# chechaohp/gan-ode

Measured on AMD Instinct MI355X. Metric: generated videos/sec (16-frame clips), higher is better.
Workload: dtype f32

## Files before the change

### gan-ode_amd/_lib.py

```python
from __future__ import annotations

import ctypes as C
import os
import sys

_HERE = os.path.dirname(os.path.abspath(__file__))
LIB_PATH = os.path.join(_HERE, "lib", "libgode.so")

i32, i64, f32, ptr = C.c_int32, C.c_int64, C.c_float, C.c_void_p
cint, u32, u64 = C.c_int, C.c_uint32, C.c_uint64

ACT_NONE, ACT_RELU, ACT_LRELU, ACT_TANH_OUT = 0, 1, 2, 3
ACT_TANH, ACT_SIGMOID = 4, 5
ACT_LRELU01 = 6
EPI_RAW, EPI_TANH = 0, 1
FPROP, DGRAD = 0, 1
PACK_BORDER = 0x100
OP_IGEMM, OP_WGRAD, OP_BN_FINALIZE, OP_BN_BWD, OP_ODE_FWD, OP_ODE_BWD, OP_BCE, OP_ADAM, OP_PACK = range(1, 10)
OP_ODERNN_FWD, OP_ODERNN_BWD, OP_BN_APPLY, OP_COL2IM = 10, 11, 12, 13
OP_SDE_FWD, OP_SDE_BWD = 14, 15
OP_CDE_FWD, OP_CDE_BWD = 16, 17
OP_WGAN = 18
OP_GRU_FWD, OP_GRU_BWD = 19, 20
OP_DNOISE = 21
# ... 37 lines not shown

class ConvGeom(C.Structure):
    _fields_ = [(n, i32) for n in "N Ci Co Di Hi Wi Do Ho Wo kd kh kw sd sh sw pd ph pw".split()]

    def key(self):
        return tuple(getattr(self, n) for n, _ in self._fields_)


class _Op(C.Structure):
    """An op of gode_run (a GODE_OPS row of gode.h): a subclass names its kind and its `int FN(const op*, stream)` entry
    point once; _STRUCTS, the prototypes, EXPORTS and run_one's dispatch all follow from the subclasses."""


class IgemmOp(_Op):
    _fields_ = [("g", ConvGeom), ("dir", i32), ("act", i32), ("epilogue", i32), ("tile", i32), ("src", ptr),
                ("wpack", ptr), ("out", ptr), ("scale", ptr), ("shift", ptr), ("stats", ptr), ("gs", i64 * 5),
                ("work", ptr), ("groups", i32), ("border", i32)]
    KIND, FN = OP_IGEMM, "gode_igemm"


class WgradOp(_Op):
    _fields_ = [("g", ConvGeom), ("act", i32), ("xform_on_y", i32), ("splits", i32), ("accumulate", i32),
                ("x", ptr), ("y", ptr), ("scale", ptr), ("shift", ptr), ("work", ptr), ("dw", ptr),
                ("co_perm", ptr), ("co_canon", i64), ("xs", i64 * 5)]
    KIND, FN = OP_WGRAD, "gode_wgrad"


class BnFinalizeOp(_Op):
    _fields_ = [("stats", ptr), ("rows", i32), ("ncols", i32), ("C", i32), ("count", i64), ("gamma", ptr),
                ("beta", ptr), ("running_mean", ptr), ("running_var", ptr), ("num_batches_tracked", ptr),
                ("mean", ptr), ("invstd", ptr), ("scale", ptr), ("shift", ptr), ("momentum", f32), ("eps", f32),
                ("training", i32), ("pad_", i32), ("groups", i32), ("rows0", i32), ("nseg", i32), ("order", i32),
                ("count1", i64), ("seg", i32 * 24), ("stats1", ptr), ("rows1", i32), ("pad3_", i32), ("batch_var", ptr)]
    KIND, FN = OP_BN_FINALIZE, "gode_bn_finalize"


class BnRunningLayer(C.Structure):
    _fields_ = [("mean", ptr), ("var", ptr), ("running_mean", ptr), ("running_var", ptr), ("num_batches_tracked", ptr),
                ("C", i32), ("pad_", i32)]


class BnRunningOp(_Op):
    _fields_ = [("layer", BnRunningLayer * BN_RUNNING_MAX), ("n", i32), ("momentum", f32)]
    KIND, FN = OP_BN_RUNNING, "gode_bn_running"


class BnBwdOp(_Op):
# ... 267 lines not shown


_OPS = _Op.__subclasses__()
_STRUCTS = {0: ConvGeom, REC_ADAM_NOISE: AdamNoiseTensor, OP_PACK: PackOp, **{st.KIND: st for st in _OPS}}

_PROTOS = {
    "gode_igemm_stats_rows": ([ptr], cint),
    "gode_igemm_stats_rows0": ([ptr], cint),
    "gode_igemm_stats_segments": ([ptr, i32, ptr], cint),
    "gode_igemm_model_cycles": ([ptr], C.c_double),
    "gode_igemm_family": ([ptr], cint),
    "gode_igemm_dead_taps": ([ptr], C.c_double),
    "gode_igemm_launch_info": ([ptr, ptr], cint),
    "gode_igemm_launch_cell": ([ptr, ptr], cint),
    "gode_igemm_work_size": ([ptr], i64),
    "gode_col2im_launch_kind": ([ptr, ptr], cint),
    "gode_video_grid_launch_kind": ([ptr, ptr], cint),
    "gode_gif_lzw_bound": ([i64], i64),
    "gode_gif_lzw": ([ptr, i64, i32, ptr, i64], i64),
    "gode_pack_size": ([ptr, cint], i64),
    "gode_pack_weights": ([ptr, cint, ptr, ptr, ptr, i32, ptr], cint),
    "gode_wgrad_work_size": ([ptr], i64),
    "gode_wgrad_auto_splits": ([ptr], cint),
    "gode_bn_bwd_work_size": ([i64, i32], i64),
    "gode_ode_bwd_work_size": ([i32], i64),
    "gode_odernn_bwd_work_size": ([i32], i64),
    "gode_odernn_sync_size": ([i32], i64),
    "gode_sde_bwd_work_size": ([i32], i64),
    "gode_cde_sync_size": ([i32], i64),
    "gode_cde_state_size": ([i32, i32], i64),
    "gode_cde_bwd_work_size": ([i32], i64),
    "gode_gru_bwd_work_size": ([i32], i64),
    "gode_ode_fwd_multi": ([ptr, i32, ptr], cint),
    "gode_ode_bwd_multi": ([ptr, i32, ptr], cint),
    "gode_odernn_fwd_multi": ([ptr, i32, ptr], cint),
    "gode_odernn_bwd_multi": ([ptr, i32, ptr], cint),
    "gode_odernn_fwd_route": ([ptr, i32, ptr], cint),
    "gode_odernn_bwd_route": ([ptr, i32, ptr], cint),
    "gode_gru_fwd_multi": ([ptr, i32, ptr], cint),
    "gode_gru_bwd_multi": ([ptr, i32, ptr], cint),
    "gode_chstats_rows": ([i64], cint),
    "gode_cbn_bwd_work_size": ([i32, i32, i32, i32], i64),
    "gode_gres_out_bwd_work_size": ([i32, i32, i32, i32, i32, i32], i64),
    "gode_fc_act_bwd_work_size": ([i64, i32], i64),
    "gode_dropout_mask": ([ptr, i64, u64, u32, f32, ptr], cint),
    "gode_scale": ([ptr, ptr, i64, f32, cint, ptr], cint),
# ... 167 lines not shown
```

### gan-ode_amd/csrc/wgrad.hip

```cpp
#include "common.h"
#include "wgrad_plan.h"

struct WgradArgs {
  gode_conv_geom g;
  const float* x; const float* y; const float* scale; const float* shift; float* work;
  int32_t xsN, xsD, xsH, xsW, xsC;
  int32_t act, xform_on_y;
  int32_t M, chunk, Kt, taps;
  FastDiv dWo, dHo, dDo;
  uint32_t x_bytes;
};

template <int WM, int WN, int TM, int TN, bool VECX, bool VECY>
__global__ void __launch_bounds__(WM* WN * 64) wgrad_kernel(const WgradArgs a) {
  constexpr int NT = WM * WN * 64, BI = WM * TM * 32, BJ = WN * TN * 32;
  static_assert(NT == 256, "loader assumes 256 threads");
  constexpr int YC = BI / 4, XC = BJ / 4;
  constexpr int YR = NT / YC, XR = NT / XC;
  constexpr int YP = 32 / YR, XP = 32 / XR;
  static_assert(YP >= 1 && XP >= 1, "tile too narrow for the loader");
  __shared__ __attribute__((aligned(16))) float smem[2 * 32 * (BI + BJ)];

  const int tid = threadIdx.x, lane = tid & 63, wave = tid >> 6;
  const int wm = wave / WN, wn = wave % WN;
// ... 329 lines not shown
      stage();
      __syncthreads();
      fetch(s + 1);
      mma_slab(0);
      __syncthreads();
    }
    stage();
    __syncthreads();
    mma_slab(0);
  }

  float* dst = a.work + (int64_t)z * g.Co * a.Kt;
  const int col0 = jblk * BJ + wn * TN * 32 + (lane & 31) * TN;
#pragma unroll
  for (int i = 0; i < TM; ++i)
#pragma unroll
    for (int r = 0; r < 16; ++r) {
      const int row = iblk * BI + wm * TM * 32 + TM * ((r & 3) + 8 * (r >> 2) + 4 * (lane >> 5)) + i;
      if (row < g.Co && col0 < a.Kt) {
        bv_t v;
#pragma unroll
        for (int j = 0; j < TN; ++j) v[j] = acc[i][j][r];
        *reinterpret_cast<bv_t*>(dst + (int64_t)row * a.Kt + col0) = v;
      }
    }
}

__global__ void __launch_bounds__(256) wgrad_thin_kernel(const WgradArgs a, int chunk_thin) {
  const gode_conv_geom& g = a.g;
  const int C4 = g.Co >> 2;
  const int CL = C4 < 64 ? C4 : 64;
  const int ML = 256 / CL;
  const int tid = threadIdx.x, cl = tid % CL, ml = tid / CL;
  const int Kt = a.Kt;
  __shared__ __attribute__((aligned(16))) float red[4][256][4];
  const float nslope = gode_act_neg_slope(a.act);
  const float xneg = a.xform_on_y ? 1.f : nslope, yneg = a.xform_on_y ? nslope : 1.f;
  const int m0 = blockIdx.x * chunk_thin;
  const int m1 = m0 + chunk_thin < a.M ? m0 + chunk_thin : a.M;
  for (int cg = 0; cg < C4; cg += CL) {
    const int c4 = cg + cl;
    const bool cok = ml < ML && c4 < C4;
    f32x4 acc[THIN_MAXKT];
#pragma unroll
    for (int j = 0; j < THIN_MAXKT; ++j) acc[j] = f32x4{0.f, 0.f, 0.f, 0.f};
    f32x4 ysc = {1, 1, 1, 1}, ysh = {0, 0, 0, 0};
// ... 261 lines not shown
#pragma unroll 8
    for (int zz = 0; zz < splits; ++zz) {
      if (VEC4) {
        const f32x4 v = *reinterpret_cast<const f32x4*>(work + (int64_t)zz * total + i);
#pragma unroll
        for (int e = 0; e < V; ++e) sd[e] += (double)v[e];
      } else {
        sd[0] += (double)work[(int64_t)zz * total + i];
      }
    }
    int co = (int)(i / Kt);
    const int j0 = (int)(i - (int64_t)co * Kt);
    if (co_perm) { co = co_perm[co]; if (co < 0) continue; }
#pragma unroll
    for (int e = 0; e < V; ++e) {
      const int j = j0 + e, tap = j / Ci, ci = j - tap * Ci;
      float* dptr = dw + ((int64_t)co * Ci + ci) * taps + tap;
      const float sv = (float)sd[e];
      *dptr = accumulate ? *dptr + sv : sv;
    }
  }
}

#define RS_LANES 16
__global__ void __launch_bounds__(256) wgrad_reduce_small_kernel(const float* work, float* dw, int Co, int Ci, int taps,
                                                                 int splits, const int32_t* co_perm, int accumulate) {
  __shared__ double red[RS_LANES][RS_OUT];
  const int Kt = Ci * taps, total = Co * Kt;
  const int o = threadIdx.x & (RS_OUT - 1), ln = threadIdx.x / RS_OUT;
  const int i = blockIdx.x * RS_OUT + o;
  double sd = 0.0;
  if (i < total) {
#pragma unroll 8
    for (int zz = ln; zz < splits; zz += RS_LANES) sd += (double)work[(int64_t)zz * total + i];
  }
  red[ln][o] = sd;
  __syncthreads();
  if (ln == 0 && i < total) {
    double tot = 0.0;
#pragma unroll
    for (int q = 0; q < RS_LANES; ++q) tot += red[q][o];
    const float sv = (float)tot;
    int co = i / Kt;
    const int j = i - co * Kt, tap = j / Ci, ci = j - tap * Ci;
    if (co_perm) { co = co_perm[co]; if (co < 0) return; }
    float* dptr = dw + ((int64_t)co * Ci + ci) * taps + tap;
    *dptr = accumulate ? *dptr + sv : sv;
  }
}


extern "C" int gode_wgrad_auto_splits(const gode_conv_geom* g) { return wgrad_auto_splits(*g); }
extern "C" int64_t gode_wgrad_work_size(const gode_wgrad_op* op) { return wgrad_work_size(op); }

#define WG_TILE_ARGS(t) WGRAD_TILES[t].WM, WGRAD_TILES[t].WN, WGRAD_TILES[t].TM, WGRAD_TILES[t].TN

extern "C" int gode_wgrad(const gode_wgrad_op* op, void* stream) {
  if (!op || !op->x || !op->y || !op->work || !op->dw) return GODE_E_ARG;
  WgradPlan P;
  const int rc = wgrad_make_plan(op, &P);
  if (rc) return rc;
  const gode_conv_geom& g = op->g;
  const WgradPatch& w = P.work.patch;
  const int splits = P.work.splits;
  WpArgs WP;
  WgradArgs& A = WP.w;
  A.g = g; A.x = op->x; A.y = op->y; A.scale = op->scale; A.shift = op->shift; A.work = op->work;
  A.xsN = P.xs[0]; A.xsD = P.xs[1]; A.xsH = P.xs[2]; A.xsW = P.xs[3]; A.xsC = P.xs[4];
  A.act = op->act; A.xform_on_y = op->xform_on_y;
  A.M = P.M; A.chunk = P.chunk; A.Kt = P.Kt; A.taps = P.taps;
  A.dWo = make_fastdiv(g.Wo); A.dHo = make_fastdiv(g.Ho); A.dDo = make_fastdiv(g.Do);
  A.x_bytes = P.x_bytes;
  if (P.path == WG_PATCH) {
    WP.RB = w.RB; WP.CB = w.CB; WP.PR = w.PR; WP.PL = w.PL; WP.LW = w.LW; WP.nseg = w.nseg; WP.dseg = make_fastdiv((uint32_t)w.nseg);
    WP.segs = w.segs; WP.segs_per_wg = w.segs_per_wg; WP.yvec = P.vy;
  }
  hipStream_t st = (hipStream_t)stream;
  const dim3 grid(P.grid_x, P.grid_y, P.grid_z), block(P.block);
#define WG_CASE_FAST(t, gl) case wgrad_fast_key(t, gl): hipLaunchKernelGGL((wgrad_fast_kernel<WG_TILE_ARGS(t), gl != 0>), grid, block, 0, st, A); break;
#define WG_CASE_GENERIC(t, vx, vy) case wgrad_generic_key(t, vx, vy): hipLaunchKernelGGL((wgrad_kernel<WG_TILE_ARGS(t), vx != 0, vy != 0>), grid, block, 0, st, A); break;
#define WG_CASE_PATCH(n, c) case wgrad_patch_key(n, c): hipLaunchKernelGGL((wgrad_patch_kernel<n, c>), grid, block, P.lds_bytes, st, WP); break;
  switch (wgrad_kernel_key(P, g.Co)) {
    WGRAD_FAST_KERNELS(WG_CASE_FAST)
    WGRAD_GENERIC_KERNELS(WG_CASE_GENERIC)
    WGRAD_PATCH_KERNELS(WG_CASE_PATCH)
    case wgrad_thin_key(): hipLaunchKernelGGL(wgrad_thin_kernel, grid, block, 0, st, A, P.chunk_thin); break;
    default: return GODE_E_SHAPE;
  }
#undef WG_CASE_FAST
#undef WG_CASE_GENERIC
#undef WG_CASE_PATCH
  GODE_LAUNCH_CHECK();
  const dim3 rgrid(P.reduce_blocks), rblock(256);
  switch (P.reduce) {
    case WG_REDUCE_SMALL:
      hipLaunchKernelGGL(wgrad_reduce_small_kernel, rgrid, rblock, 0, st, op->work, op->dw, g.Co, g.Ci, P.taps, splits, op->co_perm, op->accumulate);
      break;
    case WG_REDUCE_VEC4:
      hipLaunchKernelGGL((wgrad_reduce_kernel<true>), rgrid, rblock, 0, st, op->work, op->dw, g.Co, g.Ci, P.taps, splits, op->co_perm, op->accumulate);
      break;
    default:
      hipLaunchKernelGGL((wgrad_reduce_kernel<false>), rgrid, rblock, 0, st, op->work, op->dw, g.Co, g.Ci, P.taps, splits, op->co_perm, op->accumulate);
  }
  GODE_LAUNCH_CHECK();
  return 0;
}
```

### gan-ode_amd/csrc/wgrad_plan.h

```cpp
#pragma once
#include <stdint.h>
#include <stdlib.h>
#include "conv_geom.h"

#define THIN_MAXKT 16
#define WP_MAXB 4
#define WP_MAXE 16
#define RS_OUT 16

enum { WG_TILE_32x128 = 0, WG_TILE_64x128 = 1, WG_TILE_128x128 = 2, WG_TILE_256x128 = 3, WG_TILE_128x256 = 4, WGRAD_TILE_IDS = 5 };
struct WgradTile { int BI, BJ, WM, WN, TM, TN, waves; };
constexpr WgradTile wgrad_tile(int WM, int WN, int TM, int TN) { return WgradTile{WM * TM * 32, WN * TN * 32, WM, WN, TM, TN, WM * WN}; }
static constexpr WgradTile WGRAD_TILES[WGRAD_TILE_IDS] = {wgrad_tile(1, 4, 1, 1), wgrad_tile(2, 2, 1, 2), wgrad_tile(2, 2, 2, 2),
                                                          wgrad_tile(4, 2, 2, 2), wgrad_tile(2, 4, 2, 2)};

struct WgradKnobs { int tile; bool generic, glds; };
static const WgradKnobs& wgrad_knobs() {
  static const WgradKnobs k = [] {
    const char* t = getenv("GODE_WGRAD_TILE");
    const char* gl = getenv("GODE_WGRAD_GLDS");
    return WgradKnobs{t ? atoi(t) : 0, getenv("GODE_WGRAD_GENERIC") != nullptr, gl ? atoi(gl) != 0 : true};
  }();
  return k;
}
// ... 55 lines not shown
  const int nseg = (g.Wo + 31) / 32;
  const int64_t segs = (int64_t)g.N * g.Do * g.Ho * nseg;
  if (segs >= (1ll << 31)) return false;
  int wgs = (int)(segs / 2 < 1 ? 1 : segs / 2);
  if (wgs > 512) wgs = 512;
  *P = WgradPatch{RB, CB, PR, PL, LW, nseg, (int)segs, (int)((segs + wgs - 1) / wgs), nbw};
  return true;
}

enum { WG_PATCH = 0, WG_THIN = 1, WG_GEMM = 2 };
struct WgradWork { int32_t rule, split_tile, splits; WgradPatch patch; };
static WgradWork wgrad_plan_work(const gode_conv_geom& g, int splits, bool has_scale, bool xform_on_y, const WgradKnobs& knobs) {
  WgradWork W = {WG_GEMM, wgrad_pick_tile(g, knobs), splits, {0, 0, 0, 0, 0, 0, 0, 0, 0}};
  if (wgrad_patch_shape(g, splits > 0, has_scale && !xform_on_y, &W.patch)) {
    W.rule = WG_PATCH; W.splits = (W.patch.segs + W.patch.segs_per_wg - 1) / W.patch.segs_per_wg;
  } else if (splits <= 0 && wgrad_thin_eligible(g)) {
    W.rule = WG_THIN; W.splits = wgrad_thin_blocks(g);
  } else if (splits <= 0) {
    W.splits = wgrad_gemm_splits(g, W.split_tile);
  }
  return W;
}
static int wgrad_auto_splits(const gode_conv_geom& g) { return wgrad_gemm_splits(g, wgrad_pick_tile(g, wgrad_knobs())); }
static int64_t wgrad_work_size(const gode_wgrad_op* op) {
  const WgradWork W = wgrad_plan_work(op->g, op->splits, op->scale != nullptr, op->xform_on_y != 0, wgrad_knobs());
  return (int64_t)W.splits * op->g.Co * op->g.kd * op->g.kh * op->g.kw * op->g.Ci;
}

enum { WG_FAST = 0, WG_GENERIC = 1 };
enum { WG_REDUCE_SMALL = 0, WG_REDUCE_VEC4 = 1, WG_REDUCE_SCALAR = 2 };

struct WgradPlan {
  WgradWork work;
  int32_t path;
  int32_t tile, family;
  int32_t vx, vy, glds;
  int32_t M, taps, Kt, chunk, chunk_thin;
  int32_t grid_x, grid_y, grid_z, block, lds_bytes;
  int32_t xs[5];
  uint32_t x_bytes;
  int32_t reduce, reduce_blocks;
  int64_t work_floats;
};

#define WGRAD_FAST_KERNELS(X) X(0, 0) X(0, 1) X(1, 0) X(1, 1) X(2, 0) X(2, 1) X(3, 0) X(3, 1) X(4, 0) X(4, 1)
#define WGRAD_GENERIC_KERNELS(X) \
  X(0, 0, 0) X(0, 0, 1) X(0, 1, 0) X(0, 1, 1) X(1, 0, 0) X(1, 0, 1) X(1, 1, 0) X(1, 1, 1) X(2, 0, 0) X(2, 0, 1) X(2, 1, 0) X(2, 1, 1)
#define WGRAD_PATCH_KERNELS(X) \
  X(1, 32) X(2, 32) X(3, 32) X(4, 32) X(1, 64) X(2, 64) X(3, 64) X(4, 64) X(1, 128) X(2, 128) X(3, 128) X(4, 128)
constexpr uint32_t wgrad_key(int path, int family, int tile, int glds, int vx, int vy, int nbw, int Co) {
  return (uint32_t)path | (uint32_t)family << 2 | (uint32_t)tile << 3 | (uint32_t)glds << 6 | (uint32_t)vx << 7 | (uint32_t)vy << 8 |
         (uint32_t)nbw << 9 | (uint32_t)Co << 12;
}
constexpr uint32_t wgrad_fast_key(int tile, int glds) { return wgrad_key(WG_GEMM, WG_FAST, tile, glds, 1, 1, 0, 0); }
constexpr uint32_t wgrad_generic_key(int tile, int vx, int vy) { return wgrad_key(WG_GEMM, WG_GENERIC, tile, 0, vx, vy, 0, 0); }
constexpr uint32_t wgrad_patch_key(int nbw, int Co) { return wgrad_key(WG_PATCH, 0, 0, 0, 0, 0, nbw, Co); }
constexpr uint32_t wgrad_thin_key() { return wgrad_key(WG_THIN, 0, 0, 0, 0, 0, 0, 0); }
static uint32_t wgrad_kernel_key(const WgradPlan& P, int Co) {
  if (P.path == WG_PATCH) return wgrad_patch_key(P.work.patch.nbw, Co);
  if (P.path == WG_THIN) return wgrad_thin_key();
  return P.family == WG_FAST ? wgrad_fast_key(P.tile, P.glds) : wgrad_generic_key(P.tile, P.vx, P.vy);
}
static constexpr uint32_t WGRAD_KERNEL_KEYS[] = {
#define WG_KEY_FAST(t, gl) wgrad_fast_key(t, gl),
#define WG_KEY_GENERIC(t, vx, vy) wgrad_generic_key(t, vx, vy),
#define WG_KEY_PATCH(n, c) wgrad_patch_key(n, c),
    WGRAD_FAST_KERNELS(WG_KEY_FAST) WGRAD_GENERIC_KERNELS(WG_KEY_GENERIC) WGRAD_PATCH_KERNELS(WG_KEY_PATCH) wgrad_thin_key()};
#undef WG_KEY_FAST
#undef WG_KEY_GENERIC
#undef WG_KEY_PATCH

static int wgrad_make_plan_with(const gode_wgrad_op* op, const WgradKnobs& knobs, WgradPlan* P) {
  if (!op) return GODE_E_ARG;
  const gode_conv_geom& g = op->g;
  IgemmGeom chk;
  const int rc = gode_build_igemm_geom(g, GODE_FPROP, &chk);
  if (rc) return rc;
  int64_t xs[5];
  if (gode_strides_are_channels_last(op->xs)) {
    xs[4] = 1; xs[3] = g.Ci; xs[2] = (int64_t)g.Wi * xs[3]; xs[1] = (int64_t)g.Hi * xs[2]; xs[0] = (int64_t)g.Di * xs[1];
  } else {
    for (int i = 0; i < 5; ++i) xs[i] = op->xs[i];
  }
  const int64_t span = 1 + (int64_t)(g.N - 1) * xs[0] + (int64_t)(g.Di - 1) * xs[1] + (int64_t)(g.Hi - 1) * xs[2] +
                       (int64_t)(g.Wi - 1) * xs[3] + (int64_t)(g.Ci - 1) * xs[4];
  const int64_t M = (int64_t)g.N * g.Do * g.Ho * g.Wo;
  if (span >= (1ll << 31) || M * g.Co >= (1ll << 31)) return GODE_E_SHAPE;
  for (int i = 0; i < 5; ++i) P->xs[i] = (int32_t)xs[i];
  P->x_bytes = (span * 4 < (1ll << 31) && M * g.Co * 4 < (1ll << 31)) ? (uint32_t)(span * 4) : 0u;
  P->M = (int)M; P->taps = g.kd * g.kh * g.kw; P->Kt = P->taps * g.Ci;

  const WgradWork& W = P->work = wgrad_plan_work(g, op->splits, op->scale != nullptr, op->xform_on_y != 0, knobs);
  const int splits = W.splits;
  P->chunk = (int)(((M + splits - 1) / splits + 31) / 32 * 32);
  P->chunk_thin = 0;
  P->vx =xs[4] == 1 && g.Ci % 4 == 0 && xs[0] % 4 == 0 && xs[1] % 4 == 0 && xs[2] % 4 == 0 && xs[3] % 4 == 0 && (uintptr_t)op->x % 16 == 0;
  P->vy = g.Co % 4 == 0 && (uintptr_t)op->y % 16 == 0;
  P->tile = -1; P->family = -1; P->glds = 0;
  P->grid_x = splits; P->grid_y = 1; P->grid_z = 1; P->block = 256; P->lds_bytes = 0;
  if (W.rule == WG_PATCH) {
    P->path = WG_PATCH;
    P->lds_bytes = 2 * (W.patch.PR * W.patch.PL + 32 * g.Co + 4) * 4;
  } else if (W.rule == WG_THIN && P->vy) {
    P->path = WG_THIN;
    P->chunk_thin = (int)((M + splits - 1) / splits);
  } else {
    P->path = WG_GEMM;
    const bool fast = P->vx && P->vy && !knobs.generic;
    P->family = fast ? WG_FAST : WG_GENERIC;
    P->tile = WGRAD_TILES[W.split_tile].waves == 8 && !fast ? WG_TILE_128x128 : W.split_tile;
    const bool glds_on = WGRAD_TILES[P->tile].waves == 8 || knobs.glds;
    P->glds = fast && glds_on && op->scale == nullptr && op->act == GODE_ACT_NONE && P->x_bytes != 0;
    P->grid_x = gode_ceil_div(P->Kt, WGRAD_TILES[P->tile].BJ); P->grid_y = gode_ceil_div(g.Co, WGRAD_TILES[P->tile].BI); P->grid_z = splits;
    P->block = WGRAD_TILES[P->tile].waves * 64;
  }

  const int64_t total = (int64_t)g.Co * P->Kt;
  if ((total <= 8192 || (P->path == WG_PATCH && total <= 32768)) && splits >= 16) {
    P->reduce = WG_REDUCE_SMALL;
    P->reduce_blocks = (int)((total + RS_OUT - 1) / RS_OUT);
  } else {
    const bool v4 = P->Kt % 4 == 0 && (uintptr_t)op->work % 16 == 0;
    P->reduce = v4 ? WG_REDUCE_VEC4 : WG_REDUCE_SCALAR;
    const int64_t blocks = (total / (v4 ? 4 : 1) + 255) / 256;
    P->reduce_blocks = (int)(blocks > 4096 ? 4096 : (blocks < 1 ? 1 : blocks));
  }
  P->work_floats = (int64_t)splits * total;
  return 0;
}
static int wgrad_make_plan(const gode_wgrad_op* op, WgradPlan* P) { return wgrad_make_plan_with(op, wgrad_knobs(), P); }
```

### gan-ode_amd/engine.py

```python
from __future__ import annotations

import ctypes as C
import os
from dataclasses import dataclass
from typing import List, Optional, Sequence

import numpy as np
import torch

from . import _lib as L

BORDER_TAKE_DEAD_TAPS = 0.06
BORDER_TAKE_TILES_PER_SLOT = 2.0


def border_value(g) -> int:
    lib = L.lib()
    if lib.gode_igemm_dead_taps(C.byref(L.IgemmOp(g=g, dir=L.DGRAD, tile=0))) < BORDER_TAKE_DEAD_TAPS:
        return 1
    info = (C.c_int32 * 4)()
    L.check(lib.gode_igemm_launch_info(C.byref(L.IgemmOp(g=g, dir=L.DGRAD, tile=0, border=2)), info))
    return 2 if info[0] and info[2] >= BORDER_TAKE_TILES_PER_SLOT * info[3] else 1


def make_geom(N, Ci, Co, xi, yo, k, s, p) -> L.ConvGeom:
    return L.ConvGeom(N, Ci, Co, xi[0], xi[1], xi[2], yo[0], yo[1], yo[2], k[0], k[1], k[2], s[0], s[1], s[2],
                      p[0], p[1], p[2])


def conv_out(i, k, s, p):
    return (i + 2 * p - k) // s + 1


def dptr(t: Optional[torch.Tensor]):
    return None if t is None else t.data_ptr()


def stream_ptr():
    return torch.cuda.current_stream().cuda_stream


def tensor_version(t):
    return (t._version, getattr(t, "_gode_ver", 0), t.data_ptr())


# ... 652 lines not shown
    def _build_bwd(self, need_input_grad: bool, need_param_grad: bool = True, training: bool = True):
        lib = L.lib()
        f32 = dict(dtype=torch.float32, device=self.device)
        if self.g is None:
            self.g = [torch.empty(s.out_dims(), **f32) for s in self.specs]
            self.g_in = None
        ops, patch = [], {"dw": [], "dgamma": [], "dbeta": []}
        bpacks = []
        wg_work = 0
        bn_work = 0
        last = self.specs[-1]
        readers = patch["gout_readers"] = []
        if last.epilogue == L.EPI_TANH:
            M = self._count(self.nl - 1)
            op = L.BnBwdOp(g=dptr(self.g[-1]), y=None, M=M, C=last.out_dims()[4], act=L.ACT_TANH_OUT)
            patch["tanh"] = op
            readers.append((op, "gin"))
            ops.append(op)
        for l in range(self.nl - 1, -1, -1):
            s, p = self.specs[l], self.params[l]
            rev = L.DGRAD if s.fwd_dir == L.FPROP else L.FPROP
            sc, sh, act = self._in_xform(l)
            src = self._in_src(l)
            if self.groups == 2 and l == 0:
                hg = self._half_geom(s.geom)
                half = self.g[0].numel() // 2
                pair = []
                for k in range(2):
                    pair.append(L.WgradOp(g=hg, act=act, xform_on_y=0, splits=0, accumulate=0,
                                          x=None if self.x0n is None else self.x0n.data_ptr() + 4 * (self.x0n.numel() // 2) * k,
                                          y=self.g[0].data_ptr() + 4 * half * k, scale=dptr(sc), shift=dptr(sh)))
                if need_param_grad:
                    for k, wk in enumerate(pair):
                        wg_work = max(wg_work, lib.gode_wgrad_work_size(C.byref(wk)))
                        patch["dw"].append((l, wk, k == 1))
                        ops.append(wk)
                    patch["wgrad0"], patch["wgrad0b"] = pair
                if need_input_grad:
                    raise NotImplementedError("a grouped stack does not return input gradients")
                continue
            if self._last_parts and l == self.nl - 1:
                if s.fwd_dir != L.DGRAD or "tanh" not in patch:
                    raise NotImplementedError("split stack: per-part output layer is a transposed convolution with tanh")
                per_in, per_out, Cs = int(np.prod(s.in_dims()[1:])), int(np.prod(s.out_dims()[1:])), sc.numel() // 2
                if need_param_grad:
                    for n, img0, k in ((self.split, 0, 0), (s.geom.N - self.split, self.split, 1)):
                        wk = L.WgradOp(g=self._part_geom(s.geom, n), act=act, xform_on_y=1, splits=0, accumulate=0,
                                       x=self.g[l].data_ptr() + 4 * img0 * per_out, y=src.data_ptr() + 4 * img0 * per_in,
                                       scale=sc.data_ptr() + 4 * Cs * k, shift=sh.data_ptr() + 4 * Cs * k, co_perm=dptr(s.co_perm))
                        wg_work = max(wg_work, lib.gode_wgrad_work_size(C.byref(wk)))
                        patch["dw"].append((l, wk, k == 1))
                        ops.append(wk)
                w = None
            elif s.fwd_dir == L.FPROP:
                w = L.WgradOp(g=s.geom, act=act, xform_on_y=0, splits=0, accumulate=0, x=dptr(src), y=dptr(self.g[l]),
                              scale=dptr(sc), shift=dptr(sh), co_perm=dptr(s.co_perm))
            else:
                w = L.WgradOp(g=s.geom, act=act, xform_on_y=1, splits=0, accumulate=0, x=dptr(self.g[l]), y=dptr(src),
                              scale=dptr(sc), shift=dptr(sh), co_perm=dptr(s.co_perm))
            if need_param_grad and w is not None:
                wg_work = max(wg_work, lib.gode_wgrad_work_size(C.byref(w)))
                patch["dw"].append((l, w, False))
                if l == 0:
                    patch["wgrad0"] = w
                if l == self.nl - 1 and "tanh" not in patch:
                    readers.append((w, "y" if s.fwd_dir == L.FPROP else "x"))
                ops.append(w)
            if l > 0 or need_input_grad:
                rank1 = self._rank1_head(l, "tanh" in patch)
                tg = self._tail_as_gemm() if l == 0 else None
                dst = self.g_in if l == 0 else self.g[l - 1]
                if tg is not None:
                    g = s.geom
                    wp = self._shared_pack(0, "tail_gemm", lib.gode_pack_size(C.byref(tg), L.DGRAD))
                    bpacks.append((0, "tail_gemm", L.PackOp(g=tg, dir=L.DGRAD, co_canon=0, w=dptr(p.weight), wpack=dptr(wp),
                                                            co_perm=dptr(s.co_perm))))
                    if getattr(self, "_tail_cols", None) is None:
                        self._tail_cols = torch.empty(tg.N * g.kd * g.kh * g.kw * g.Ci, **f32)
                    ops.append(L.IgemmOp(g=tg, dir=L.DGRAD, act=L.ACT_NONE, epilogue=L.EPI_RAW, tile=0, src=dptr(self.g[0]),
                                         wpack=dptr(wp), out=dptr(self._tail_cols)))
                    c2i = L.Col2imOp(cols=dptr(self._tail_cols), out=None, N=g.N, Hi=g.Ho, Wi=g.Wo, Ho=g.Hi, Wo=g.Wi, C=g.Ci,
                                     kh=g.kh, kw=g.kw, sh=g.sh, sw=g.sw, ph=g.ph, pw=g.pw, epilogue=L.EPI_RAW,
# ... 167 lines not shown
```

### include/gode.h

```cpp
#ifndef GODE_H
#define GODE_H
#include <stdint.h>
#ifdef __cplusplus
extern "C" {
#endif

#define GODE_VERSION 105

enum { GODE_OK = 0, GODE_E_ARG = -1, GODE_E_SHAPE = -2, GODE_E_KIND = -3 };
enum { GODE_ACT_NONE = 0, GODE_ACT_RELU = 1, GODE_ACT_LRELU = 2,
       GODE_ACT_TANH_OUT = 3 ,
       GODE_ACT_TANH = 4, GODE_ACT_SIGMOID = 5 ,
       GODE_ACT_LRELU01 = 6  };
enum { GODE_EPI_RAW = 0, GODE_EPI_TANH = 1 };
enum { GODE_FPROP = 0, GODE_DGRAD = 1 };
enum { GODE_PACK_BORDER = 0x100 };

typedef struct gode_conv_geom {
  int32_t N, Ci, Co;
  int32_t Di, Hi, Wi;
  int32_t Do, Ho, Wo;
  int32_t kd, kh, kw;
  int32_t sd, sh, sw;
  int32_t pd, ph, pw;
// ... 18 lines not shown
int gode_igemm_stats_rows(const gode_igemm_op* op);
int gode_igemm_stats_rows0(const gode_igemm_op* op);
int gode_igemm_stats_segments(const gode_igemm_op* op, int32_t split_images, int32_t* seg);
double gode_igemm_model_cycles(const gode_igemm_op* op);
int gode_igemm_family(const gode_igemm_op* op);
int gode_igemm_launch_cell(const gode_igemm_op* op, int32_t* cell);
double gode_igemm_dead_taps(const gode_igemm_op* op);
int gode_igemm_launch_info(const gode_igemm_op* op, int32_t* info);
int64_t gode_pack_size(const gode_conv_geom* g, int dir);
int gode_pack_weights(const gode_conv_geom* g, int dir, const float* w, float* wpack, const int32_t* co_perm,
                      int32_t co_canon, void* stream);

typedef struct gode_wgrad_op {
  gode_conv_geom g;
  int32_t act, xform_on_y, splits, accumulate;
  const float* x;
  const float* y;
  const float* scale;
  const float* shift;
  float* work;
  float* dw;
  const int32_t* co_perm; int64_t co_canon;
  int64_t xs[5];
} gode_wgrad_op;
int gode_wgrad(const gode_wgrad_op* op, void* stream);
int64_t gode_wgrad_work_size(const gode_wgrad_op* op);
int gode_wgrad_auto_splits(const gode_conv_geom* g);

typedef struct gode_bn_finalize_op {
  const float* stats; int32_t rows, ncols, C; int64_t count;
  const float* gamma; const float* beta;
  float* running_mean; float* running_var; int64_t* num_batches_tracked;
  float* mean; float* invstd; float* scale; float* shift;
  float momentum, eps; int32_t training, pad_;
  int32_t groups, rows0;
  int32_t nseg, order; int64_t count1; int32_t seg[24];
  const float* stats1; int32_t rows1, pad3_;
  float* batch_var;
} gode_bn_finalize_op;
int gode_bn_finalize(const gode_bn_finalize_op* op, void* stream);

#define GODE_BN_RUNNING_MAX 8
typedef struct gode_bn_running_layer {
  const float* mean; const float* var; float* running_mean; float* running_var; int64_t* num_batches_tracked;
  int32_t C, pad_;
} gode_bn_running_layer;
typedef struct gode_bn_running_op {
  gode_bn_running_layer layer[8];
  int32_t n; float momentum;
// ... 428 lines not shown
```

Measured before the change: 43050.

## Add cell-major wgrad kernel that skips dead spatial cells per K tile

Adds a weight-gradient GEMM variant that splits the reduction by output spatial cell instead of by flat M. For each K-column tile it works out the rectangle of output cells whose taps touch valid input, so border cells whose taps only hit padding are never loaded. Work is balanced across workgroups with a cost model, and a matching per-tile reduction kernel follows. The engine turns it on only for plain (no scale or activation) 2D layers whose chosen tile index is high enough. The price is a larger workspace and more planning code, and the speedup depends on how much padding waste the affected layers actually have.

```diff
diff --git a/gan-ode_amd/_lib.py b/gan-ode_amd/_lib.py
--- a/gan-ode_amd/_lib.py
+++ b/gan-ode_amd/_lib.py
@@ -83,7 +83,7 @@
 class WgradOp(_Op):
     _fields_ = [("g", ConvGeom), ("act", i32), ("xform_on_y", i32), ("splits", i32), ("accumulate", i32),
                 ("x", ptr), ("y", ptr), ("scale", ptr), ("shift", ptr), ("work", ptr), ("dw", ptr),
-                ("co_perm", ptr), ("co_canon", i64), ("xs", i64 * 5)]
+                ("co_perm", ptr), ("co_canon", i64), ("xs", i64 * 5), ("cell_major", i32), ("pad_", i32)]
     KIND, FN = OP_WGRAD, "gode_wgrad"
 
 
@@ -397,6 +397,7 @@
     "gode_pack_weights": ([ptr, cint, ptr, ptr, ptr, i32, ptr], cint),
     "gode_wgrad_work_size": ([ptr], i64),
     "gode_wgrad_auto_splits": ([ptr], cint),
+    "gode_wgrad_launch_info": ([ptr, ptr], cint),
     "gode_bn_bwd_work_size": ([i64, i32], i64),
     "gode_ode_bwd_work_size": ([i32], i64),
     "gode_odernn_bwd_work_size": ([i32], i64),
diff --git a/gan-ode_amd/csrc/wgrad.hip b/gan-ode_amd/csrc/wgrad.hip
--- a/gan-ode_amd/csrc/wgrad.hip
+++ b/gan-ode_amd/csrc/wgrad.hip
@@ -375,6 +375,139 @@
 #pragma unroll
         for (int j = 0; j < TN; ++j) v[j] = acc[i][j][r];
         *reinterpret_cast<bv_t*>(dst + (int64_t)row * a.Kt + col0) = v;
+      }
+    }
+}
+
+struct WgcArgs {
+  WgradArgs w;
+  int32_t ntj, spc, planes, pad_;
+  WgcTile t[WGC_MAXJ + 1];
+};
+
+template <int WM, int WN, int TM, int TN>
+__global__ void __launch_bounds__(WM* WN * 64) wgrad_cell_kernel(const WgcArgs c) {
+  constexpr int NT = WM * WN * 64, BI = WM * TM * 32, BJ = WN * TN * 32;
+  constexpr int YC = BI / 4, XC = BJ / 4, YR = NT / YC, XR = NT / XC, YP = 32 / YR, XP = 32 / XR;
+  static_assert(YP >= 1 && XP >= 1, "tile too narrow for the loader");
+  static_assert(YC % 64 == 0 || 64 % YC == 0, "loader pass must be lane-linear");
+  constexpr int BUF = 32 * (BI + BJ);
+  __shared__ __attribute__((aligned(16))) float smem[2 * BUF];
+  const WgradArgs& a = c.w;
+  const gode_conv_geom& g = a.g;
+  const int tid = threadIdx.x, lane = tid & 63, wave = tid >> 6;
+  const int wm = wave / WN, wn = wave % WN;
+  const int bx = blockIdx.x, iblk = blockIdx.y;
+  int jblk = 0;
+  while (jblk + 1 < c.ntj && (int)c.t[jblk + 1].wg0 <= bx) ++jblk;
+  const int h0 = c.t[jblk].h0, w0 = c.t[jblk].w0, w1 = c.t[jblk].w1, rw = w1 - w0;
+  const int L = (c.t[jblk].h1 - h0) * rw * c.spc;
+  int t0, t1;
+  wgc_slab_range(L, (int)c.t[jblk + 1].wg0 - (int)c.t[jblk].wg0, bx - (int)c.t[jblk].wg0, &t0, &t1);
+  const int nslab = t1 - t0;
+
+  const int ych = tid % YC, yr0 = tid / YC, xch = tid % XC, xr0 = tid / XC;
+  const int co0 = iblk * BI + ych * 4, j0 = jblk * BJ + xch * 4;
+  const bool yok = co0 < g.Co, xok = j0 < a.Kt;
+  const int tap = xok ? j0 / g.Ci : 0;
+  const int xci = xok ? j0 - tap * g.Ci : 0;
+  const int xkw = tap % g.kw, xkh = (tap / g.kw) % g.kh, xkd = tap / (g.kw * g.kh);
+
+  const int wave_u = __builtin_amdgcn_readfirstlane(wave);
+  const BufRsrc rsrcX = make_buf_rsrc(a.x, a.x_bytes);
+  const int cells = g.Ho * g.Wo;
+  int yvoff[YP];
+#pragma unroll
+  for (int p = 0; p < YP; ++p) yvoff[p] = yok ? ((yr0 + p * YR) * cells * g.Co + co0) * 4 : (int)0x80000000;
+  int ps = 0, qh = h0, qw = w0;
+  if (nslab > 0) {
+    const int cell = t0 / c.spc;
+    ps = t0 - cell * c.spc; qh = h0 + cell / rw; qw = w0 + cell % rw;
+  }
+  auto dma = [&](int buf) {
+    float* Ys = smem + buf * BUF + wave_u * 256;
+    float* Xs = smem + buf * BUF + 32 * BI + wave_u * 256;
+    const int left = c.planes - ps * 32;
+    const int rows = left > 32 ? 32 : left;
+    const BufRsrc rsrcY = make_buf_rsrc(a.y + ((int64_t)ps * 32 * cells + qh * g.Wo + qw) * g.Co,
+                                        (uint32_t)((rows - 1) * cells * g.Co + g.Co) * 4u);
+#pragma unroll
+    for (int p = 0; p < YP; ++p) buf_dma16(rsrcY, Ys + p * YR * BI, yvoff[p], 0);
+    const int ih = qh * g.sh - g.ph + xkh, iw = qw * g.sw - g.pw + xkw;
+    const bool sok = xok && (unsigned)ih < (unsigned)g.Hi && (unsigned)iw < (unsigned)g.Wi;
+    const int soff = ih * a.xsH + iw * a.xsW + xci;
+#pragma unroll
+    for (int p = 0; p < XP; ++p) {
+      const int r = xr0 + p * XR;
+      const uint32_t pl = (uint32_t)(ps * 32 + r);
+      const uint32_t img = fdiv(pl, a.dDo);
+      const int id = (int)(pl - img * g.Do) * g.sd - g.pd + xkd;
+      const bool ok = sok && r < rows && (unsigned)id < (unsigned)g.Di;
+      buf_dma16(rsrcX, Xs + p * XR * BJ, ok ? ((int)img * a.xsN + id * a.xsD + soff) * 4 : (int)0x80000000, 0);
+    }
+    if (++ps == c.spc) {
+      ps = 0;
+      if (++qw == w1) { qw = w0; ++qh; }
+    }
+  };
+
+  f32x16 acc[TM][TN];
+#pragma unroll
+  for (int i = 0; i < TM; ++i)
+#pragma unroll
+    for (int j = 0; j < TN; ++j)
+#pragma unroll
+      for (int r = 0; r < 16; ++r) acc[i][j][r] = 0.f;
+
+  typedef float __attribute__((ext_vector_type(TM))) av_t;
+  typedef float __attribute__((ext_vector_type(TN))) bv_t;
+  const int fr = lane & 31, fh = lane >> 5;
+  const float* Yr = smem + fh * BI + wm * TM * 32 + fr * TM;
+  const float* Xr = smem + 32 * BI + fh * BJ + wn * TN * 32 + fr * TN;
+  av_t fa[2][4]; bv_t fb[2][4];
+  auto frag = [&](int buf, int kg, int set) {
+#pragma unroll
+    for (int q = 0; q < 4; ++q) {
+      fa[set][q] = *reinterpret_cast<const av_t*>(Yr + buf * BUF + (kg * 4 + q) * 2 * BI);
+      fb[set][q] = *reinterpret_cast<const bv_t*>(Xr + buf * BUF + (kg * 4 + q) * 2 * BJ);
+    }
+  };
+  auto mma = [&](int set) {
+#pragma unroll
+    for (int q = 0; q < 4; ++q)
+#pragma unroll
+      for (int i = 0; i < TM; ++i)
+#pragma unroll
+        for (int j = 0; j < TN; ++j) acc[i][j] = __builtin_amdgcn_mfma_f32_32x32x2f32(fa[set][q][i], fb[set][q][j], acc[i][j], 0, 0, 0);
+  };
+  if (nslab > 0) {
+    dma(0);
+    __syncthreads();
+    frag(0, 0, 0);
+    for (int s = 0; s < nslab; ++s) {
+      const int buf = s & 1;
+      if (s + 1 < nslab) dma(buf ^ 1);
+      frag(buf, 1, 1); __builtin_amdgcn_sched_barrier(0); mma(0); __builtin_amdgcn_sched_barrier(0);
+      frag(buf, 2, 0); __builtin_amdgcn_sched_barrier(0); mma(1); __builtin_amdgcn_sched_barrier(0);
+      frag(buf, 3, 1); __builtin_amdgcn_sched_barrier(0); mma(0); __builtin_amdgcn_sched_barrier(0);
+      __syncthreads();
+      frag(buf ^ 1, 0, 0);
+      __builtin_amdgcn_sched_barrier(0); mma(1); __builtin_amdgcn_sched_barrier(0);
+    }
+  }
+
+  float* dst = a.work + (int64_t)bx * g.Co * BJ;
+  const int colt = wn * TN * 32 + (lane & 31) * TN;
+#pragma unroll
+  for (int i = 0; i < TM; ++i)
+#pragma unroll
+    for (int r = 0; r < 16; ++r) {
+      const int row = iblk * BI + wm * TM * 32 + TM * ((r & 3) + 8 * (r >> 2) + 4 * (lane >> 5)) + i;
+      if (row < g.Co && jblk * BJ + colt < a.Kt) {
+        bv_t v;
+#pragma unroll
+        for (int j = 0; j < TN; ++j) v[j] = acc[i][j][r];
+        *reinterpret_cast<bv_t*>(dst + (int64_t)row * BJ + colt) = v;
       }
     }
 }
@@ -682,6 +815,42 @@
   }
 }
 
+struct WgcPrefix { uint16_t wg0[WGC_MAXJ + 1]; };
+template <bool VEC4>
+__global__ void __launch_bounds__(256) wgrad_cell_reduce_kernel(const float* work, float* dw, int Co, int Ci, int taps, int BJ,
+                                                                const WgcPrefix pf, const int32_t* co_perm, int accumulate) {
+  constexpr int V = VEC4 ? 4 : 1;
+  const int Kt = Ci * taps, jblk = blockIdx.y;
+  const int wg_begin = pf.wg0[jblk], wg_end = pf.wg0[jblk + 1];
+  const int i = (blockIdx.x * 256 + threadIdx.x) * V;
+  if (i >= Co * BJ) return;
+  int co = i / BJ;
+  const int jt = i - co * BJ, j0 = jblk * BJ + jt;
+  if (j0 >= Kt) return;
+  const float* src = work + (int64_t)co * BJ + jt;
+  double sd[V];
+#pragma unroll
+  for (int e = 0; e < V; ++e) sd[e] = 0.0;
+#pragma unroll 8
+  for (int wg = wg_begin; wg < wg_end; ++wg) {
+    if (VEC4) {
+      const f32x4 v = *reinterpret_cast<const f32x4*>(src + (int64_t)wg * Co * BJ);
+#pragma unroll
+      for (int e = 0; e < V; ++e) sd[e] += (double)v[e];
+    } else {
+      sd[0] += (double)src[(int64_t)wg * Co * BJ];
+    }
+  }
+  if (co_perm) { co = co_perm[co]; if (co < 0) return; }
+#pragma unroll
+  for (int e = 0; e < V; ++e) {
+    const int j = j0 + e, tap = j / Ci, ci = j - tap * Ci;
+    float* dptr = dw + ((int64_t)co * Ci + ci) * taps + tap;
+    const float sv = (float)sd[e];
+    *dptr = accumulate ? *dptr + sv : sv;
+  }
+}
+
 #define RS_LANES 16
 __global__ void __launch_bounds__(256) wgrad_reduce_small_kernel(const float* work, float* dw, int Co, int Ci, int taps,
                                                                  int splits, const int32_t* co_perm, int accumulate) {
@@ -712,6 +881,18 @@
 
 extern "C" int gode_wgrad_auto_splits(const gode_conv_geom* g) { return wgrad_auto_splits(*g); }
 extern "C" int64_t gode_wgrad_work_size(const gode_wgrad_op* op) { return wgrad_work_size(op); }
+extern "C" int gode_wgrad_launch_info(const gode_wgrad_op* op, int32_t* info) {
+  if (!info) return GODE_E_ARG;
+  WgradPlan P;
+  const int rc = wgrad_make_plan(op, &P);
+  if (rc) return rc;
+  const int plain_load = P.path == WG_GEMM ? P.chunk / 32 : 0;
+  info[0] = P.cell.on; info[1] = P.tile; info[2] = P.grid_x * P.grid_y * P.grid_z;
+  info[3] = P.cell.on ? P.cell.max_load : plain_load;
+  info[4] = (int32_t)((P.cell.on ? P.cell.live_slabs : (int64_t)plain_load * info[2]) & 0x7fffffff);
+  info[5] = plain_load; info[6] = 0; info[7] = 0;
+  return 0;
+}
 
 #define WG_TILE_ARGS(t) WGRAD_TILES[t].WM, WGRAD_TILES[t].WN, WGRAD_TILES[t].TM, WGRAD_TILES[t].TN
 
@@ -737,22 +918,41 @@
   }
   hipStream_t st = (hipStream_t)stream;
   const dim3 grid(P.grid_x, P.grid_y, P.grid_z), block(P.block);
+  WgcArgs WC;
+  WgcPrefix PF;
+  if (P.cell.on) {
+    WC.w = A; WC.ntj = P.cell.ntj; WC.spc = P.cell.spc; WC.planes = P.cell.planes; WC.pad_ = 0;
+    for (int j = 0; j <= WGC_MAXJ; ++j) {
+      WC.t[j] = P.cell.t[j <= P.cell.ntj ? j : P.cell.ntj];
+      PF.wg0[j] = WC.t[j].wg0;
+    }
+  }
 #define WG_CASE_FAST(t, gl) case wgrad_fast_key(t, gl): hipLaunchKernelGGL((wgrad_fast_kernel<WG_TILE_ARGS(t), gl != 0>), grid, block, 0, st, A); break;
 #define WG_CASE_GENERIC(t, vx, vy) case wgrad_generic_key(t, vx, vy): hipLaunchKernelGGL((wgrad_kernel<WG_TILE_ARGS(t), vx != 0, vy != 0>), grid, block, 0, st, A); break;
 #define WG_CASE_PATCH(n, c) case wgrad_patch_key(n, c): hipLaunchKernelGGL((wgrad_patch_kernel<n, c>), grid, block, P.lds_bytes, st, WP); break;
+#define WG_CASE_CELL(t) case wgrad_cell_key(t): hipLaunchKernelGGL((wgrad_cell_kernel<WG_TILE_ARGS(t)>), grid, block, 0, st, WC); break;
   switch (wgrad_kernel_key(P, g.Co)) {
     WGRAD_FAST_KERNELS(WG_CASE_FAST)
     WGRAD_GENERIC_KERNELS(WG_CASE_GENERIC)
     WGRAD_PATCH_KERNELS(WG_CASE_PATCH)
+    WGRAD_CELL_KERNELS(WG_CASE_CELL)
     case wgrad_thin_key(): hipLaunchKernelGGL(wgrad_thin_kernel, grid, block, 0, st, A, P.chunk_thin); break;
     default: return GODE_E_SHAPE;
   }
 #undef WG_CASE_FAST
 #undef WG_CASE_GENERIC
 #undef WG_CASE_PATCH
+#undef WG_CASE_CELL
   GODE_LAUNCH_CHECK();
-  const dim3 rgrid(P.reduce_blocks), rblock(256);
+  const dim3 rgrid(P.reduce_blocks, P.cell.on ? P.cell.ntj : 1), rblock(256);
+  const int cBJ = P.cell.on ? WGRAD_TILES[P.tile].BJ : 0;
   switch (P.reduce) {
+    case WG_REDUCE_CELL_VEC4:
+      hipLaunchKernelGGL((wgrad_cell_reduce_kernel<true>), rgrid, rblock, 0, st, op->work, op->dw, g.Co, g.Ci, P.taps, cBJ, PF, op->co_perm, op->accumulate);
+      break;
+    case WG_REDUCE_CELL_SCALAR:
+      hipLaunchKernelGGL((wgrad_cell_reduce_kernel<false>), rgrid, rblock, 0, st, op->work, op->dw, g.Co, g.Ci, P.taps, cBJ, PF, op->co_perm, op->accumulate);
+      break;
     case WG_REDUCE_SMALL:
       hipLaunchKernelGGL(wgrad_reduce_small_kernel, rgrid, rblock, 0, st, op->work, op->dw, g.Co, g.Ci, P.taps, splits, op->co_perm, op->accumulate);
       break;
diff --git a/gan-ode_amd/csrc/wgrad_plan.h b/gan-ode_amd/csrc/wgrad_plan.h
--- a/gan-ode_amd/csrc/wgrad_plan.h
+++ b/gan-ode_amd/csrc/wgrad_plan.h
@@ -101,13 +101,120 @@
   return W;
 }
 static int wgrad_auto_splits(const gode_conv_geom& g) { return wgrad_gemm_splits(g, wgrad_pick_tile(g, wgrad_knobs())); }
+
+static int64_t wgrad_resolve_xs(const gode_wgrad_op* op, int64_t xs[5]) {
+  const gode_conv_geom& g = op->g;
+  if (gode_strides_are_channels_last(op->xs)) {
+    xs[4] = 1; xs[3] = g.Ci; xs[2] = (int64_t)g.Wi * xs[3]; xs[1] = (int64_t)g.Hi * xs[2]; xs[0] = (int64_t)g.Di * xs[1];
+  } else {
+    for (int i = 0; i < 5; ++i) xs[i] = op->xs[i];
+  }
+  return 1 + (int64_t)(g.N - 1) * xs[0] + (int64_t)(g.Di - 1) * xs[1] + (int64_t)(g.Hi - 1) * xs[2] + (int64_t)(g.Wi - 1) * xs[3] +
+         (int64_t)(g.Ci - 1) * xs[4];
+}
+
+#define WGC_MAXJ 64
+struct WgcTile { uint16_t wg0, h0, h1, w0, w1, pad_; };
+struct WgradCell {
+  int32_t on;
+  int32_t tile, nti, ntj;
+  int32_t spc, planes;
+  int32_t grid_x;
+  int32_t max_load, plain_load;
+  int64_t live_slabs;
+  int64_t work_floats;
+  WgcTile t[WGC_MAXJ + 1];
+};
+
+static void wgc_live(int k, int s, int p, int I, int O, int* lo, int* hi) {
+  const int a = p - k, b = I - 1 + p - k;
+  int l = a > 0 ? (a + s - 1) / s : 0, h = b >= 0 ? b / s + 1 : 0;
+  if (h > O) h = O;
+  if (l >= h) { l = 0; h = 0; }
+  *lo = l; *hi = h;
+}
+static void wgc_tile_rect(const gode_conv_geom& g, int j0, int j1, WgcTile* t) {
+  int h0 = g.Ho, h1 = 0, w0 = g.Wo, w1 = 0;
+  for (int tap = j0 / g.Ci; tap <= (j1 - 1) / g.Ci; ++tap) {
+    int a, b, c, d;
+    wgc_live((tap / g.kw) % g.kh, g.sh, g.ph, g.Hi, g.Ho, &a, &b);
+    wgc_live(tap % g.kw, g.sw, g.pw, g.Wi, g.Wo, &c, &d);
+    if (a == b || c == d) continue;
+    h0 = a < h0 ? a : h0; h1 = b > h1 ? b : h1; w0 = c < w0 ? c : w0; w1 = d > w1 ? d : w1;
+  }
+  if (h1 <= h0 || w1 <= w0) h0 = h1 = w0 = w1 = 0;
+  t->h0 = (uint16_t)h0; t->h1 = (uint16_t)h1; t->w0 = (uint16_t)w0; t->w1 = (uint16_t)w1; t->pad_ = 0;
+}
+GODE_HD void wgc_slab_range(int L, int S, int s, int* t0, int* t1) {
+  *t0 = (int)((int64_t)L * s / S); *t1 = (int)((int64_t)L * (s + 1) / S);
+}
+
+#define WGC_SLAB_OVERHEAD (114.0 / 32.0)
+static bool wgrad_cell_plan(const gode_wgrad_op* op, const WgradKnobs& knobs, const WgradWork& W, WgradCell* C) {
+  const gode_conv_geom& g = op->g;
+  C->on = 0;
+  if (g.N < 1 || g.Ci < 1 || g.Co < 1 || g.Do < 1 || g.Ho < 1 || g.Wo < 1 || g.kh < 1 || g.kw < 1 || g.sh < 1 || g.sw < 1) return false;
+  if ((op->cell_major != 1 && op->cell_major != 2) || op->splits > 0 || op->scale != nullptr || op->act != GODE_ACT_NONE || W.rule != WG_GEMM || knobs.generic)
+    return false;
+  int64_t xs[5];
+  const int64_t span = wgrad_resolve_xs(op, xs), M = (int64_t)g.N * g.Do * g.Ho * g.Wo;
+  if (span * 4 >= (1ll << 31) || M * g.Co * 4 >= (1ll << 31)) return false;
+  if (xs[4] != 1 || g.Ci % 4 != 0 || g.Co % 4 != 0 || xs[0] % 4 != 0 || xs[1] % 4 != 0 || xs[2] % 4 != 0 || xs[3] % 4 != 0) return false;
+  const WgradTile& T = WGRAD_TILES[W.split_tile];
+  if (T.waves != 8 && !knobs.glds) return false;
+  const int Kt = g.kd * g.kh * g.kw * g.Ci, planes = g.N * g.Do;
+  const int ntj = gode_ceil_div(Kt, T.BJ), nti = gode_ceil_div(g.Co, T.BI), spc = (planes + 31) / 32;
+  if (planes < 32 || ntj > WGC_MAXJ || g.Ho > 65535 || g.Wo > 65535) return false;
+  if (32ll * g.Ho * g.Wo * g.Co * 4 >= (1ll << 31)) return false;
+  int L[WGC_MAXJ], maxL = 1;
+  int64_t sumL = 0;
+  for (int j = 0; j < ntj; ++j) {
+    const int j1 = (j + 1) * T.BJ < Kt ? (j + 1) * T.BJ : Kt;
+    wgc_tile_rect(g, j * T.BJ, j1, &C->t[j]);
+    L[j] = (C->t[j].h1 - C->t[j].h0) * (C->t[j].w1 - C->t[j].w0) * spc;
+    sumL += L[j];
+    if (L[j] > maxL) maxL = L[j];
+  }
+  const bool w8 = T.waves == 8;
+  auto price = [&](int64_t wgs, int load) {
+    const double rounds = (double)((wgs + 255) / 256), overlap = (wgs >= 512 || w8) ? 1.0 : 0.92;
+    return rounds * ((double)load + WGC_SLAB_OVERHEAD) / overlap;
+  };
+  int bestT = 0; double best = 1e300;
+  for (int tl = 2; tl <= (maxL < 2 ? 2 : maxL); ++tl) {
+    int64_t wgs = 0; int load = 0;
+    for (int j = 0; j < ntj; ++j) {
+      const int S = L[j] > tl ? (L[j] + tl - 1) / tl : 1, ld = (L[j] + S - 1) / S;
+      wgs += S; if (ld > load) load = ld;
+    }
+    if (wgs > 65535 / nti) continue;
+    const double c = price(wgs * nti, load);
+    if (c < best - 1e-12) { best = c; bestT = tl; }
+  }
+  if (!bestT) return false;
+  const int plain_load = (int)((((M + W.splits - 1) / W.splits) + 31) / 32);
+  if (op->cell_major != 2 && best >= 0.97 * price((int64_t)nti * ntj * W.splits, plain_load)) return false;
+  int wg = 0, load = 0;
+  for (int j = 0; j < ntj; ++j) {
+    const int S = L[j] > bestT ? (L[j] + bestT - 1) / bestT : 1, ld = (L[j] + S - 1) / S;
+    C->t[j].wg0 = (uint16_t)wg; wg += S; if (ld > load) load = ld;
+  }
+  WgcTile& end = C->t[ntj];
+  end.wg0 = (uint16_t)wg; end.h0 = end.h1 = end.w0 = end.w1 = end.pad_ = 0;
+  C->on = 1; C->tile = W.split_tile; C->nti = nti; C->ntj = ntj; C->spc = spc; C->planes = planes; C->grid_x = wg;
+  C->max_load = load; C->plain_load = plain_load; C->live_slabs = sumL * nti; C->work_floats = (int64_t)wg * g.Co * T.BJ;
+  return true;
+}
+
 static int64_t wgrad_work_size(const gode_wgrad_op* op) {
   const WgradWork W = wgrad_plan_work(op->g, op->splits, op->scale != nullptr, op->xform_on_y != 0, wgrad_knobs());
-  return (int64_t)W.splits * op->g.Co * op->g.kd * op->g.kh * op->g.kw * op->g.Ci;
+  const int64_t plain = (int64_t)W.splits * op->g.Co * op->g.kd * op->g.kh * op->g.kw * op->g.Ci;
+  WgradCell C;
+  return wgrad_cell_plan(op, wgrad_knobs(), W, &C) && C.work_floats > plain ? C.work_floats : plain;
 }
 
 enum { WG_FAST = 0, WG_GENERIC = 1 };
-enum { WG_REDUCE_SMALL = 0, WG_REDUCE_VEC4 = 1, WG_REDUCE_SCALAR = 2 };
+enum { WG_REDUCE_SMALL = 0, WG_REDUCE_VEC4 = 1, WG_REDUCE_SCALAR = 2, WG_REDUCE_CELL_VEC4 = 3, WG_REDUCE_CELL_SCALAR = 4 };
 
 struct WgradPlan {
   WgradWork work;
@@ -120,9 +227,11 @@
   uint32_t x_bytes;
   int32_t reduce, reduce_blocks;
   int64_t work_floats;
+  WgradCell cell;
 };
 
 #define WGRAD_FAST_KERNELS(X) X(0, 0) X(0, 1) X(1, 0) X(1, 1) X(2, 0) X(2, 1) X(3, 0) X(3, 1) X(4, 0) X(4, 1)
+#define WGRAD_CELL_KERNELS(X) X(0) X(1) X(2) X(3) X(4)
 #define WGRAD_GENERIC_KERNELS(X) \
   X(0, 0, 0) X(0, 0, 1) X(0, 1, 0) X(0, 1, 1) X(1, 0, 0) X(1, 0, 1) X(1, 1, 0) X(1, 1, 1) X(2, 0, 0) X(2, 0, 1) X(2, 1, 0) X(2, 1, 1)
 #define WGRAD_PATCH_KERNELS(X) \
@@ -135,16 +244,21 @@
 constexpr uint32_t wgrad_generic_key(int tile, int vx, int vy) { return wgrad_key(WG_GEMM, WG_GENERIC, tile, 0, vx, vy, 0, 0); }
 constexpr uint32_t wgrad_patch_key(int nbw, int Co) { return wgrad_key(WG_PATCH, 0, 0, 0, 0, 0, nbw, Co); }
 constexpr uint32_t wgrad_thin_key() { return wgrad_key(WG_THIN, 0, 0, 0, 0, 0, 0, 0); }
+constexpr uint32_t wgrad_cell_key(int tile) { return wgrad_fast_key(tile, 1) | 1u << 24; }
 static uint32_t wgrad_kernel_key(const WgradPlan& P, int Co) {
   if (P.path == WG_PATCH) return wgrad_patch_key(P.work.patch.nbw, Co);
   if (P.path == WG_THIN) return wgrad_thin_key();
+  if (P.cell.on) return wgrad_cell_key(P.tile);
   return P.family == WG_FAST ? wgrad_fast_key(P.tile, P.glds) : wgrad_generic_key(P.tile, P.vx, P.vy);
 }
 static constexpr uint32_t WGRAD_KERNEL_KEYS[] = {
 #define WG_KEY_FAST(t, gl) wgrad_fast_key(t, gl),
 #define WG_KEY_GENERIC(t, vx, vy) wgrad_generic_key(t, vx, vy),
 #define WG_KEY_PATCH(n, c) wgrad_patch_key(n, c),
-    WGRAD_FAST_KERNELS(WG_KEY_FAST) WGRAD_GENERIC_KERNELS(WG_KEY_GENERIC) WGRAD_PATCH_KERNELS(WG_KEY_PATCH) wgrad_thin_key()};
+#define WG_KEY_CELL(t) wgrad_cell_key(t),
+    WGRAD_FAST_KERNELS(WG_KEY_FAST) WGRAD_GENERIC_KERNELS(WG_KEY_GENERIC) WGRAD_PATCH_KERNELS(WG_KEY_PATCH) WGRAD_CELL_KERNELS(WG_KEY_CELL)
+    wgrad_thin_key()};
+#undef WG_KEY_CELL
 #undef WG_KEY_FAST
 #undef WG_KEY_GENERIC
 #undef WG_KEY_PATCH
@@ -156,13 +270,7 @@
   const int rc = gode_build_igemm_geom(g, GODE_FPROP, &chk);
   if (rc) return rc;
   int64_t xs[5];
-  if (gode_strides_are_channels_last(op->xs)) {
-    xs[4] = 1; xs[3] = g.Ci; xs[2] = (int64_t)g.Wi * xs[3]; xs[1] = (int64_t)g.Hi * xs[2]; xs[0] = (int64_t)g.Di * xs[1];
-  } else {
-    for (int i = 0; i < 5; ++i) xs[i] = op->xs[i];
-  }
-  const int64_t span = 1 + (int64_t)(g.N - 1) * xs[0] + (int64_t)(g.Di - 1) * xs[1] + (int64_t)(g.Hi - 1) * xs[2] +
-                       (int64_t)(g.Wi - 1) * xs[3] + (int64_t)(g.Ci - 1) * xs[4];
+  const int64_t span = wgrad_resolve_xs(op, xs);
   const int64_t M = (int64_t)g.N * g.Do * g.Ho * g.Wo;
   if (span >= (1ll << 31) || M * g.Co >= (1ll << 31)) return GODE_E_SHAPE;
   for (int i = 0; i < 5; ++i) P->xs[i] = (int32_t)xs[i];
@@ -205,6 +313,20 @@
     P->reduce_blocks = (int)(blocks > 4096 ? 4096 : (blocks < 1 ? 1 : blocks));
   }
   P->work_floats = (int64_t)splits * total;
+  P->cell.on = 0;
+  if (op->cell_major != 0) {
+    WgradCell Cm;
+    if (wgrad_cell_plan(op, knobs, W, &Cm)) {
+      if (Cm.work_floats > P->work_floats) P->work_floats = Cm.work_floats;
+      if (P->path == WG_GEMM && P->family == WG_FAST && P->glds && P->tile == Cm.tile) {
+        P->cell = Cm;
+        P->grid_x = Cm.grid_x; P->grid_y = Cm.nti; P->grid_z = 1;
+        const bool v4 = (uintptr_t)op->work % 16 == 0;
+        P->reduce = v4 ? WG_REDUCE_CELL_VEC4 : WG_REDUCE_CELL_SCALAR;
+        P->reduce_blocks = (int)(((int64_t)g.Co * WGRAD_TILES[P->tile].BJ / (v4 ? 4 : 1) + 255) / 256);
+      }
+    }
+  }
   return 0;
 }
 static int wgrad_make_plan(const gode_wgrad_op* op, WgradPlan* P) { return wgrad_make_plan_with(op, wgrad_knobs(), P); }
diff --git a/gan-ode_amd/engine.py b/gan-ode_amd/engine.py
--- a/gan-ode_amd/engine.py
+++ b/gan-ode_amd/engine.py
@@ -21,6 +21,21 @@
     info = (C.c_int32 * 4)()
     L.check(lib.gode_igemm_launch_info(C.byref(L.IgemmOp(g=g, dir=L.DGRAD, tile=0, border=2)), info))
     return 2 if info[0] and info[2] >= BORDER_TAKE_TILES_PER_SLOT * info[3] else 1
+
+
+CELL_MAJOR_TAKE_FROM_TILE = 3
+
+
+def cell_major_value(g, plain: bool) -> int:
+    knob = os.environ.get("GODE_WGRAD_CELL_MAJOR", "")
+    if not plain or knob == "0":
+        return 0
+    if knob == "2":
+        return 2
+    info = (C.c_int32 * 8)()
+    probe = L.WgradOp(g=g, act=L.ACT_NONE, splits=0, x=4096, y=4096, work=4096, dw=4096, cell_major=2)
+    L.check(L.lib().gode_wgrad_launch_info(C.byref(probe), info))
+    return 2 if info[0] and info[1] >= CELL_MAJOR_TAKE_FROM_TILE and g.Do == 1 else 0
 
 
 def make_geom(N, Ci, Co, xi, yo, k, s, p) -> L.ConvGeom:
@@ -719,6 +734,7 @@
             rev = L.DGRAD if s.fwd_dir == L.FPROP else L.FPROP
             sc, sh, act = self._in_xform(l)
             src = self._in_src(l)
+            plain = sc is None and act == L.ACT_NONE
             if self.groups == 2 and l == 0:
                 hg = self._half_geom(s.geom)
                 half = self.g[0].numel() // 2
@@ -726,7 +742,8 @@
                 for k in range(2):
                     pair.append(L.WgradOp(g=hg, act=act, xform_on_y=0, splits=0, accumulate=0,
                                           x=None if self.x0n is None else self.x0n.data_ptr() + 4 * (self.x0n.numel() // 2) * k,
-                                          y=self.g[0].data_ptr() + 4 * half * k, scale=dptr(sc), shift=dptr(sh)))
+                                          y=self.g[0].data_ptr() + 4 * half * k, scale=dptr(sc), shift=dptr(sh),
+                                          cell_major=cell_major_value(hg, plain)))
                 if need_param_grad:
                     for k, wk in enumerate(pair):
                         wg_work = max(wg_work, lib.gode_wgrad_work_size(C.byref(wk)))
@@ -751,10 +768,10 @@
                 w = None
             elif s.fwd_dir == L.FPROP:
                 w = L.WgradOp(g=s.geom, act=act, xform_on_y=0, splits=0, accumulate=0, x=dptr(src), y=dptr(self.g[l]),
-                              scale=dptr(sc), shift=dptr(sh), co_perm=dptr(s.co_perm))
+                              scale=dptr(sc), shift=dptr(sh), co_perm=dptr(s.co_perm), cell_major=cell_major_value(s.geom, plain))
             else:
                 w = L.WgradOp(g=s.geom, act=act, xform_on_y=1, splits=0, accumulate=0, x=dptr(self.g[l]), y=dptr(src),
-                              scale=dptr(sc), shift=dptr(sh), co_perm=dptr(s.co_perm))
+                              scale=dptr(sc), shift=dptr(sh), co_perm=dptr(s.co_perm), cell_major=cell_major_value(s.geom, plain))
             if need_param_grad and w is not None:
                 wg_work = max(wg_work, lib.gode_wgrad_work_size(C.byref(w)))
                 patch["dw"].append((l, w, False))
diff --git a/include/gode.h b/include/gode.h
--- a/include/gode.h
+++ b/include/gode.h
@@ -64,9 +64,11 @@
   float* dw;
   const int32_t* co_perm; int64_t co_canon;
   int64_t xs[5];
+  int32_t cell_major, pad_;
 } gode_wgrad_op;
 int gode_wgrad(const gode_wgrad_op* op, void* stream);
 int64_t gode_wgrad_work_size(const gode_wgrad_op* op);
+int gode_wgrad_launch_info(const gode_wgrad_op* op, int32_t* info);
 int gode_wgrad_auto_splits(const gode_conv_geom* g);
 
 typedef struct gode_bn_finalize_op {
```

Result: no change. 42950 (-0.2%).
